# jizongFox/MI-based-Regularized-Semi-supervised-Segmentation

Measured on AMD Instinct MI355X. Metric: images/sec (UNet+IIC fwd/bwd) ACDC 256^2, higher is better.
Workload: dtype bf16; 1 GPU; udaiic train step, ACDC-shaped 1x256x256 4-class slices, LB=UB=16 per GPU, taps Conv5/Up_conv3/Up_conv2, K=20 x 5 sub-heads, paddings [1,3] (BASELINE configs[1]); mi_precision=f16f8, global_batch=32, parallelism=dp1, launch_tape=True, tape_ops=170, tape_replays_in_run=449

## Files before the change

include/miseg_hip.h:

```cpp
#ifndef MISEG_HIP_H
#define MISEG_HIP_H

#include <stdint.h>

#ifdef __cplusplus
extern "C" {
#endif

#define MISEG_F32 0
#define MISEG_BF16 1
#define MISEG_F16 2

#define MISEG_OK 0
#define MISEG_E_INVALID (-1)
#define MISEG_E_LAUNCH (-2)

int miseg_version(void);
const char* miseg_last_error(void);
int miseg_stream_wait_stream(void* waiter, void* producer);

int64_t miseg_tape_begin(void);
int miseg_tape_end(int64_t tape);
int miseg_tape_free(int64_t tape);
int64_t miseg_tape_mark(int64_t tape);
// ... 34 lines not shown
                        const float* grad_raw, const float* scale, float* gx, float* gy, int accumulate, int precision,
                        void* ws, int64_t ws_bytes);
int64_t miseg_iic_local_bwd_ws_bytes(int64_t K, int64_t pad, int64_t P);
int64_t miseg_iic_out_joint_ws_bytes(int64_t N, int64_t C, int64_t H, int64_t W, int64_t pad, int64_t P);
int miseg_iic_out_joint_fwd(void* stream, const float* a, const float* b, const int32_t* flips, int64_t N, int64_t C, int64_t H,
                            int64_t W, int64_t pad, const int32_t* win, int64_t P, float* raw, void* ws, int64_t ws_bytes);
int miseg_iic_out_bwd(void* stream, const float* a, const float* b, const int32_t* flips, int64_t N, int64_t C, int64_t H, int64_t W,
                      int64_t pad, const int32_t* win, int64_t P, const float* grad_raw, const float* scale, float* ga, float* gb,
                      int accumulate);
int miseg_iic_local_joint_fwd_heads(void* stream, const float* probs, int64_t S, int64_t UB, int64_t K, int64_t H, int64_t W,
                                    int64_t pad, const int32_t* win, int64_t P, float* raw, void* ws, int64_t ws_bytes,
                                    int precision);
int miseg_iic_local_bwd_heads(void* stream, const float* probs, int64_t S, int64_t UB, int64_t K, int64_t H, int64_t W,
                              int64_t pad, const int32_t* win, int64_t P, const float* grad_raw, const float* scale,
                              float* gprob, int accumulate, int precision, void* ws, int64_t ws_bytes);
int64_t miseg_iic_local_planes_bytes(int64_t S, int64_t UB, int64_t K, int64_t H, int64_t W, int64_t pad);
int miseg_iic_local_make_planes(void* stream, const float* probs, int64_t S, int64_t UB, int64_t K, int64_t H, int64_t W, int64_t pad,
                                void* planes, int64_t planes_bytes);
int miseg_iic_local_joint_fwd_heads_planes(void* stream, const float* probs, int64_t S, int64_t UB, int64_t K, int64_t H, int64_t W,
                                           int64_t pad, const int32_t* win, int64_t P, float* raw, void* ws, int64_t ws_bytes,
                                           void* planes, int64_t planes_bytes);
int miseg_iic_local_bwd_heads_planes(void* stream, const void* planes, int64_t planes_bytes, int64_t S, int64_t UB, int64_t K, int64_t H,
                                     int64_t W, int64_t pad, const int32_t* win, int64_t P, const float* grad_raw, const float* scale,
                                     float* gprob, int accumulate, void* ws, int64_t ws_bytes);

int miseg_iic_global_fwd(void* stream, const float* x, const float* y, int64_t S, int64_t N, int64_t K,
                         float lamb, float* loss, float* loss_no_lamb, float* joint);
int miseg_iic_global_bwd(void* stream, const float* x, const float* y, int64_t S, int64_t N, int64_t K,
                         float lamb, const float* upstream, float* gx, float* gy);
int miseg_iic_global_fwd_pair(void* stream, const float* prob, int64_t S, int64_t N, int64_t K, float lamb, float* loss,
// ... 223 lines not shown
```

mi-based-regularized-semi-supervised-segmentation_amd/csrc/api.hip:

```cpp
#include <stdarg.h>

#include "common.h"

namespace miseg_core {
static thread_local char g_err[512] = "";
char* last_error_buf() { return g_err; }
int fail(int code, const char* fmt, ...) {
    va_list ap;
    va_start(ap, fmt);
    vsnprintf(g_err, sizeof(g_err), fmt, ap);
    va_end(ap);
    return code;
}
}

extern "C" int miseg_version(void) { return 406; }
extern "C" const char* miseg_last_error(void) { return miseg::last_error_buf(); }

namespace miseg_core {
static hipEvent_t next_fork_event() {
    constexpr int kRing = 256, kDev = 16;
    struct Ring { hipEvent_t ev[kRing]; int made = 0, next = 0; };
    static thread_local Ring rings[kDev];
    int dev = 0;
    if (hipGetDevice(&dev) != hipSuccess || dev < 0 || dev >= kDev) return nullptr;
    Ring& r = rings[dev];
    constexpr unsigned flags = hipEventDisableTiming | hipEventDisableSystemFence;
    if (r.made < kRing) {
        if (hipEventCreateWithFlags(&r.ev[r.made], flags) != hipSuccess) return nullptr;
        ++r.made;
    }
// ... 17 lines not shown
```

mi-based-regularized-semi-supervised-segmentation_amd/csrc/mi_local.h:

```cpp
#pragma once
#include "common.h"

namespace miseg {

constexpr int kThreads = 256;
constexpr int kLdsBudget = 156 * 1024;

struct JointGeom {
    int N, K, H, W, pad, T, Mdim;
    int RB, WB, RW;
    int WX, RBY;
    int planeX, planeY;
    int P, G;
    int tilesM, sb, tps;
    int S;
    long long hs;
};

constexpr int kJT = 512;

template <int MT, int NT, int ROLE>
struct TileSet {
    static constexpr int SPLIT = (MT * NT + 1) / 2;
    static constexpr bool mine(int m, int n) { return ((m * NT + n) < SPLIT) == (ROLE == 0); }
// ... 53 lines not shown
#ifdef __HIPCC__
__device__ __forceinline__ unsigned pack_fp8x4(float a, float b, float c, float d) {
    int w = __builtin_amdgcn_cvt_pk_fp8_f32(a, b, 0, false);
    w = __builtin_amdgcn_cvt_pk_fp8_f32(c, d, w, true);
    return (unsigned)w;
}

__device__ __forceinline__ void split_quad(const float* v, qu32x2& h16, unsigned& l8, unsigned& h8) {
    const qh2_t h01 = {(_Float16)v[0], (_Float16)v[1]}, h23 = {(_Float16)v[2], (_Float16)v[3]};
    h16 = qu32x2{__builtin_bit_cast(unsigned, h01), __builtin_bit_cast(unsigned, h23)};
    l8 = pack_fp8x4((v[0] - (float)h01[0]) * 1048576.f, (v[1] - (float)h01[1]) * 1048576.f, (v[2] - (float)h23[0]) * 1048576.f,
                    (v[3] - (float)h23[1]) * 1048576.f);
    h8 = pack_fp8x4(v[0] * 256.f, v[1] * 256.f, v[2] * 256.f, v[3] * 256.f);
}

#endif

struct MiPlanes {
    unsigned char *p16, *p8l, *p8h;
};
constexpr int64_t kPlaneSlack = 4096;
static inline int64_t mi_planes_bytes(int64_t maps, int64_t HW) { return maps * HW * 88 + 4 * kPlaneSlack; }
static inline MiPlanes mi_planes(unsigned char* base, int64_t maps, int64_t HW) {
    if (!base) return MiPlanes{nullptr, nullptr, nullptr};
    unsigned char* p16 = base + kPlaneSlack;
    unsigned char* p8l = p16 + maps * HW * 40 + kPlaneSlack;
    return MiPlanes{p16, p8l, p8l + maps * HW * 24 + kPlaneSlack};
}
int launch_make_planes(hipStream_t st, const float* probs, int64_t maps, int64_t HW, unsigned char* planes);
size_t local_bwd_f8_ws_bytes(int64_t K, int64_t pad, int64_t P);
int launch_local_bwd_f8(hipStream_t st, const float* x, const float* y, int64_t S, int64_t hs, int64_t N, int64_t K, int64_t H, int64_t W,
                        int64_t pad, const int32_t* win, int64_t P, const float* grad_raw, const float* scale, float* gx, float* gy,
                        int accumulate, void* ws, const unsigned char* planes);

int launch_local_bwd_rows(hipStream_t st, const float* x, const float* y, int64_t S, int64_t hs, int64_t N, int64_t K, int64_t H, int64_t W,
                          int64_t pad, const int32_t* win, int64_t P, const float* grad_raw, const float* scale, float* gx, float* gy,
                          int accumulate, void* ws, int nterms, const unsigned char* planes = nullptr);

}
```

mi-based-regularized-semi-supervised-segmentation_amd/csrc/mi_local.hip:

```cpp
#include "mi_local.h"

namespace miseg {

template <int MT, int NT, int ROLE>
__device__ __forceinline__ void joint_fwd_body(const float* __restrict__ x, const float* __restrict__ y,
                                               const float* __restrict__ mask, const JointGeom& g,
                                               const int32_t* __restrict__ win, float* __restrict__ partials, float* lds) {
    typedef TileSet<MT, NT, ROLE> TS;
    float* Xs = lds;
    float* Ys = lds + (size_t)g.K * g.planeX;
    const int tid = threadIdx.x, lane = tid & 63, pair = tid >> 7;
    const int l15 = lane & 15, kq = lane >> 4;
    const int slot = blockIdx.y;
    const int sn = slot % g.sb, sm = (slot / g.sb) % g.sb, p = slot / (g.sb * g.sb);
    const int mtu = min(g.tps, g.tilesM - sm * g.tps), ntu = min(g.tps, g.tilesM - sn * g.tps);
    const int h0 = win[p * 4 + 0], h1 = win[p * 4 + 1], w0 = win[p * 4 + 2], w1 = win[p * 4 + 3];
    const int tr = (h1 - h0 + g.RB - 1) / g.RB, tc = (w1 - w0 + g.WB - 1) / g.WB;
    const int nItems = g.N * tr * tc;

    int aoff[MT], boff[NT];
#pragma unroll
    for (int mt = 0; mt < MT; ++mt) {
        int m = min((sm * g.tps + mt) * 16 + l15, g.Mdim - 1);
        aoff[mt] = (m % g.K) * g.planeX + (m / g.K) + kq;
// ... 95 lines not shown
                                                             const int32_t* __restrict__ win, float* __restrict__ partials) {
    extern __shared__ __attribute__((aligned(16))) float lds[];
    if (__builtin_amdgcn_readfirstlane(threadIdx.x >> 6) & 1) joint_fwd_body<MT, NT, 1>(x, y, mask, g, win, partials, lds);
    else joint_fwd_body<MT, NT, 0>(x, y, mask, g, win, partials, lds);
}

__global__ __launch_bounds__(256) void joint_reduce_kernel(const float* __restrict__ partials, JointGeom g, int MTmax, float* __restrict__ raw) {
    const int TT = g.T * g.T, KK = g.K * g.K;
    const int Dn = MTmax * 16, Dsz = Dn * Dn;
    reduce_partials_block(partials, g.G, (size_t)Dsz, g.P * TT * KK, raw, [=](int e) {
        const int j = e % g.K, i = (e / g.K) % g.K, b = (e / KK) % g.T, a = (e / (KK * g.T)) % g.T, p = e / (KK * TT);
        const int m = b * g.K + i, c = a * g.K + j;
        const int sm = m / (g.tps * 16), sn = c / (g.tps * 16);
        return ((size_t)((p * g.sb + sm) * g.sb + sn) * g.G) * Dsz + (size_t)(m - sm * g.tps * 16) * Dn + (c - sn * g.tps * 16);
    });
}

__device__ __forceinline__ float loss_displacement(const float* __restrict__ Rg, float mn, int K, int TT, float lamda, float* Pw,
                                                   float* Gw, float* colv, float* rowv, float* __restrict__ grad_d, int lane) {
    const int KK = K * K;
    const float eps = 1e-16f;
    float* Rw = rowv + 3 * K;
    for (int e = lane; e < KK; e += 64) Rw[e] = Rg[e];
    __builtin_amdgcn_wave_barrier();
    __threadfence_block();
    const float* R = Rw;
    float z = 0.f;
    for (int e = lane; e < KK; e += 64) z += (R[e] - mn) + eps;
    z = wave_sum(z);
    for (int e = lane; e < KK; e += 64) {
        int i = e / K, j = e % K;
        float q = ((R[e] - mn) + eps) / z, qt = ((R[j * K + i] - mn) + eps) / z;
        Pw[e] = (q + qt) / 2.0f;
    }
    __builtin_amdgcn_wave_barrier();
    __threadfence_block();
    if (K <= 32) {
        const int c = lane & 31;
        if (c < K) {
            float v = 0.f;
            if (lane < 32) { for (int t = 0; t < K; ++t) v += Pw[t * K + c]; }
            else { for (int t = 0; t < K; ++t) v += Pw[c * K + t]; }
            float* o = lane < 32 ? colv : rowv;
            o[c] = logf(v + eps);
            o[2 * K + c] = v / (v + eps);
        }
    } else {
        for (int c = lane; c < K; c += 64) {
            float cs = 0.f, rs = 0.f;
            for (int t = 0; t < K; ++t) { cs += Pw[t * K + c]; rs += Pw[c * K + t]; }
            colv[c] = logf(cs + eps), colv[2 * K + c] = cs / (cs + eps);
            rowv[c] = logf(rs + eps), rowv[2 * K + c] = rs / (rs + eps);
        }
    }
    __builtin_amdgcn_wave_barrier();
    __threadfence_block();
    float part = 0.f;
    for (int e = lane; e < KK; e += 64) {
        int i = e / K, j = e % K;
        float ps = Pw[e];
        float lp = logf(ps + eps), lc = colv[j], lr = rowv[i];
        part += ps * (lp - lamda * lc - lamda * lr);
        Gw[e] = -(lp + ps / (ps + eps) - lamda * (lc + colv[2 * K + j]) - lamda * (lr + rowv[2 * K + i])) / (float)TT;
    }
    const float term = -wave_sum(part);
    __builtin_amdgcn_wave_barrier();
    __threadfence_block();
    float sdot = 0.f;
    for (int e = lane; e < KK; e += 64) {
        int i = e / K, j = e % K;
        float gq = (Gw[e] + Gw[j * K + i]) / 2.0f;
        float q = ((R[e] - mn) + eps) / z;
        sdot += gq * q;
    }
    sdot = wave_sum(sdot);
    for (int e = lane; e < KK; e += 64) {
        int i = e / K, j = e % K;
        float gq = (Gw[e] + Gw[j * K + i]) / 2.0f;
        grad_d[e] = (gq - sdot) / z;
    }
    __builtin_amdgcn_wave_barrier();
    __threadfence_block();
    return term;
}

__global__ __launch_bounds__(1024) void local_loss_kernel(const float* __restrict__ raw_all, int K, int T, float lamda,
                                                          float* __restrict__ loss, float* __restrict__ grad_all) {
    extern __shared__ __attribute__((aligned(16))) float sm[];
    __shared__ float red[17];
    const int KK = K * K, TT = T * T, nw = blockDim.x >> 6, wid = threadIdx.x >> 6, lane = threadIdx.x & 63;
    const float* raw = raw_all + (size_t)blockIdx.x * TT * KK;
    float* grad = grad_all + (size_t)blockIdx.x * TT * KK;
    float* Pw = sm + (size_t)wid * (3 * KK + 4 * K);
    float* Gw = Pw + KK;
    float* colv = Gw + KK;
    float* rowv = colv + K;
    float mn = 3.4e38f;
    for (int e = threadIdx.x; e < TT * KK; e += blockDim.x) mn = fminf(mn, raw[e]);
// ... 520 lines not shown
                                           float* loss, float* grad_raw, void* ws, int64_t ws_bytes) {
    MISEG_TAPE(miseg_iic_local_loss_fwd_ws, stream, raw, K, pad, P, lamda, loss, grad_raw, ws, ws_bytes);
    MISEG_REQUIRE(raw && loss && grad_raw && ws, "iic_local_loss_fwd_ws: null pointer");
    MISEG_REQUIRE(K > 0 && K <= 64 && pad >= 0 && P > 0, "iic_local_loss_fwd_ws: bad shape");
    MISEG_REQUIRE(ws_bytes >= miseg_iic_local_loss_ws_bytes(pad, P), "iic_local_loss_fwd_ws: workspace too small");
    const int T = 2 * (int)pad + 1;
    const size_t ldsb = (size_t)(3 * K * K + 4 * K) * 4;
    hipLaunchKernelGGL(local_loss_disp_kernel, dim3((unsigned)P, (unsigned)(T * T)), dim3(1024), ldsb, as_stream(stream), raw, (int)K, T,
                       lamda, (float*)ws, grad_raw);
    MISEG_LAUNCH_CHECK("local_loss_disp_kernel");
    hipLaunchKernelGGL(local_loss_finish_kernel, dim3((unsigned)P), dim3(64), 0, as_stream(stream), (const float*)ws, T * T, loss);
    MISEG_LAUNCH_CHECK("local_loss_finish_kernel");
    return MISEG_OK;
}

extern "C" int miseg_iic_local_loss_fwd(void* stream, const float* raw, int64_t K, int64_t pad, int64_t P, float lamda,
                                        float* loss, float* grad_raw) {
    MISEG_TAPE(miseg_iic_local_loss_fwd, stream, raw, K, pad, P, lamda, loss, grad_raw);
    MISEG_REQUIRE(raw && loss && grad_raw, "iic_local_loss_fwd: null pointer");
    MISEG_REQUIRE(K > 0 && K <= 64 && pad >= 0 && P > 0, "iic_local_loss_fwd: bad shape");
    const int T = 2 * (int)pad + 1;
    const size_t ldsb = (size_t)16 * (3 * K * K + 4 * K) * 4;
    MISEG_REQUIRE(ldsb <= (size_t)kLdsBudget, "iic_local_loss_fwd: K too large");
    hipFuncSetAttribute((const void*)local_loss_kernel, hipFuncAttributeMaxDynamicSharedMemorySize, (int)ldsb);
    hipLaunchKernelGGL(local_loss_kernel, dim3((unsigned)P), dim3(1024), ldsb, as_stream(stream), raw, (int)K, T, lamda, loss,
                       grad_raw);
    MISEG_LAUNCH_CHECK("local_loss_kernel");
    return MISEG_OK;
}

// ... 69 lines not shown
```

mi-based-regularized-semi-supervised-segmentation_amd/csrc/mi_local_bwd_f8.hip:

```cpp
#include "mi_local.h"

#ifndef MISEG_F8_D1
#define MISEG_F8_D1 1
#endif
#ifndef MISEG_F8_BQ
#define MISEG_F8_BQ 1
#endif
#ifndef MISEG_F8_EDGE1
#define MISEG_F8_EDGE1 1
#endif
#ifndef MISEG_F8_STAMP
#define MISEG_F8_STAMP 0
#endif
#ifndef MISEG_F8_STORE_AUX
#define MISEG_F8_STORE_AUX 0
#endif
#ifndef MISEG_F8_ABL
#define MISEG_F8_ABL 0
#endif

namespace miseg {

template <int K, int PAD, int NT_ = 4>
struct Q3 {
// ... 1 lines not shown
    static constexpr int T = 2 * PAD + 1, REM = K - 16, RT = (T * REM + 15) / 16, MT = T + RT, MP = MT * 16;
    static constexpr int KRED = T * K, KS = (KRED + 31) / 32;
    static constexpr int CS8 = 24, CH = (T * CS8 + 31) / 32, NI = (2 * CH + 3) / 4;
    static constexpr int NT = NT_, WT = 16 * NT_, WS = WT + 2 * PAD, WSP = (WS + 7) / 8 * 8, CS = K;
    static constexpr int B16P = WSP * CS * 2;
    static constexpr int B8P = (((WT - 1) * CS8 + CH * 32 > WS * CS8 ? (WT - 1) * CS8 + CH * 32 : WS * CS8) + 15) / 16 * 16;
    static constexpr int A16B = KS * MP * 64, A8B = NI * 8 * MP * 16;
    static_assert(MP % 16 == 0, "A8 bank pattern");
};

struct Rows8Geom {
    int N, H, W, P, S, accumulate, G;
    long long hs;
};

__global__ __launch_bounds__(1024) void gexp_kernel(const float* __restrict__ grad_raw, int per, float* __restrict__ gexp) {
    const float* G = grad_raw + (size_t)blockIdx.x * per;
    float m = 0.f;
    for (int e = threadIdx.x; e < per; e += 1024) m = fmaxf(m, fabsf(G[e]));
#pragma unroll
    for (int o = 32; o > 0; o >>= 1) m = fmaxf(m, __shfl_xor(m, o, 64));
    __shared__ float red[16];
    if ((threadIdx.x & 63) == 0) red[threadIdx.x >> 6] = m;
    __syncthreads();
    if (threadIdx.x == 0) {
#pragma unroll
        for (int i = 1; i < 16; ++i) m = fmaxf(m, red[i]);
        gexp[blockIdx.x] = (m > 0.f && m < 3.0e38f) ? ldexpf(1.f, ilogbf(m)) : 1.f;
    }
}

__global__ __launch_bounds__(256) void make_planes_kernel(const float* __restrict__ probs, int maps, int HW, unsigned char* __restrict__ p16,
                                                          unsigned char* __restrict__ p8l, unsigned char* __restrict__ p8h) {
    constexpr int K = 20;
    const int pix = blockIdx.x * 256 + threadIdx.x, map = blockIdx.y;
    if (pix >= HW || map >= maps) return;
    const float* src = probs + (size_t)map * K * HW + pix;
    const size_t at = (size_t)map * HW + pix;
    unsigned h[10], l[6], g[6];
#pragma unroll
    for (int c4 = 0; c4 < K; c4 += 4) {
        const float v[4] = {src[(size_t)c4 * HW], src[(size_t)(c4 + 1) * HW], src[(size_t)(c4 + 2) * HW], src[(size_t)(c4 + 3) * HW]};
        qu32x2 hh;
// ... 6 lines not shown
    for (int i = 0; i < 5; ++i) o16[i] = qu32x2{h[2 * i], h[2 * i + 1]};
    qu32x2* ol = reinterpret_cast<qu32x2*>(p8l + at * 24);
    qu32x2* oh = reinterpret_cast<qu32x2*>(p8h + at * 24);
#pragma unroll
    for (int i = 0; i < 3; ++i) ol[i] = qu32x2{l[2 * i], l[2 * i + 1]}, oh[i] = qu32x2{g[2 * i], g[2 * i + 1]};
}

__device__ __forceinline__ void glds16(const void* gsrc, unsigned lds_dst) {
    unsigned keep;
    asm volatile("s_mov_b32 %0, m0\n\ts_mov_b32 m0, %2\n\ts_nop 0\n\tglobal_load_lds_dwordx4 %1, off\n\ts_mov_b32 m0, %0"
                 : "=&s"(keep) : "v"(gsrc), "s"(lds_dst) : "memory");
}
template <int N> __device__ __forceinline__ void wait_vm() { asm volatile("s_waitcnt vmcnt(%0)" ::"n"(N) : "memory"); }

template <int K, int PAD>
__device__ __forceinline__ float g_value(const float* __restrict__ grad_raw, int p, int dir, int m, int beta, int c, float inv) {
    typedef Q3<K, PAD> C;
    int tau, o;
    if (m < C::T * 16) { tau = m >> 4; o = m & 15; }
    else { const int rr = m - C::T * 16; tau = rr / C::REM; o = 16 + rr % C::REM; }
    if (tau >= C::T || beta >= C::T || c >= K) return 0.f;
    const int a = dir ? tau : C::T - 1 - tau, b = dir ? beta : C::T - 1 - beta;
    const float* G = grad_raw + (size_t)p * C::T * C::T * K * K + (size_t)(a * C::T + b) * K * K;
    return (dir ? G[c * K + o] : G[o * K + c]) * inv;
}

template <int K, int PAD>
__global__ void pack_g_f8_kernel(const float* __restrict__ grad_raw, const float* __restrict__ gexp, int PS, unsigned char* __restrict__ gpack) {
    typedef Q3<K, PAD> C;
    constexpr int N16 = C::KS * C::MP * 32, N8 = C::NI * 8 * C::MP * 4;
    const int total = PS * 2 * (N16 + N8);
    for (int e = blockIdx.x * blockDim.x + threadIdx.x; e < total; e += gridDim.x * blockDim.x) {
        const int sdp = e / (N16 + N8), r = e - sdp * (N16 + N8), dir = sdp & 1, p = sdp >> 1;
        const float inv = 1.f / gexp[p];
        unsigned char* base = gpack + (size_t)sdp * (C::A16B + C::A8B);
        if (r < N16) {
            const int kk = r & 31, m = (r >> 5) % C::MP, ks = r / (32 * C::MP);
            const int kred = ks * 32 + kk;
            const float v = kred < C::KRED ? g_value<K, PAD>(grad_raw, p, dir, m, kred / K, kred % K, inv) : 0.f;
            const _Float16 h = (_Float16)v;
            const size_t at = ((size_t)ks * C::MP + m) * 32 + 8 * ((kk >> 3) ^ ((0 - (m >> 2)) & 3)) + (kk & 7);
            reinterpret_cast<_Float16*>(base)[at] = h;
        } else {
            const int d = r - N16, b4 = d & 3, chunk = (d >> 6) & 7, m = ((d >> 9) % C::MT) * 16 + ((d >> 2) & 15), t = d / (512 * C::MT);
            const int j = 4 * t + (chunk >> 1), term = j / C::CH;
            float v[4];
#pragma unroll
            for (int i = 0; i < 4; ++i) {
                const int byte = (chunk & 1) * 16 + b4 * 4 + i, kk = (j % C::CH) * 32 + byte;
                float g = j < 2 * C::CH ? g_value<K, PAD>(grad_raw, p, dir, m, kk / C::CS8, kk % C::CS8, inv) : 0.f;
                const float h = (float)(_Float16)g;
                v[i] = term == 0 ? h * 128.f : (g - h) * 524288.f;
            }
            reinterpret_cast<unsigned*>(base + C::A16B)[d] = pack_fp8x4(v[0], v[1], v[2], v[3]);
        }
    }
}

template <int K, int PAD, bool ACC, int NTW, int WAVES, bool PL>
__global__ __launch_bounds__(64 * WAVES, 1) void local_bwd_f8_kernel(const float* __restrict__ x, const float* __restrict__ y, Rows8Geom g,
                                                              const int32_t* __restrict__ win,
                                                              const unsigned char* __restrict__ gpack, const float* __restrict__ gexp,
                                                              const float* __restrict__ scale, float* __restrict__ gx,
                                                              float* __restrict__ gy, unsigned long long* __restrict__ stamps,
                                                              const unsigned char* __restrict__ pl16, const unsigned char* __restrict__ pl8l,
                                                              const unsigned char* __restrict__ pl8h) {
    typedef Q3<K, PAD, NTW> C;
    constexpr int T = C::T, RT = C::RT, NT = C::NT, KS = C::KS, NI = C::NI, MP = C::MP, CS = C::CS, CS8 = C::CS8;
    constexpr int BWB = C::B16P + 2 * C::B8P;
    extern __shared__ __attribute__((aligned(16))) unsigned char ldsb[];
// ... 376 lines not shown
    if (lane == 0) {
        unsigned long long* o = stamps + ((size_t)blockIdx.x * WAVES + wv) * 8;
        o[0] = st_fetch; o[1] = st_p1; o[2] = st_p2; o[3] = st_out; o[4] = st_rows;
    }
#endif
}

size_t local_bwd_f8_ws_bytes(int64_t K, int64_t pad, int64_t P) {
    if (K != 20 || pad != 3) return 0;
    typedef Q3<20, 3> C;
    return (size_t)256 + (size_t)((P * 4 + 255) / 256 * 256) + (size_t)P * 2 * (C::A16B + C::A8B) + (MISEG_F8_STAMP ? 256 * 8 * 64 : 0);
}

bool local_bwd_f8_supported(int64_t K, int64_t pad) { return K == 20 && pad == 3; }

int launch_local_bwd_f8(hipStream_t st, const float* x, const float* y, int64_t S, int64_t hs, int64_t N, int64_t K, int64_t H, int64_t W,
                        int64_t pad, const int32_t* win, int64_t P, const float* grad_raw, const float* scale, float* gx, float* gy,
                        int accumulate, void* ws, const unsigned char* planes) {
    typedef Q3<20, 3, 4> C;
    constexpr int WAVES = 8;
    Rows8Geom g{(int)N, (int)H, (int)W, (int)P, (int)S, accumulate, 256, (long long)hs};
    const int PS = (int)(P * S);
    float* gexp = reinterpret_cast<float*>(ws);
    unsigned char* gpack = reinterpret_cast<unsigned char*>(ws) + (size_t)((PS * 4 + 255) / 256 * 256);
    hipLaunchKernelGGL(gexp_kernel, dim3(PS), dim3(1024), 0, st, grad_raw, C::T * C::T * 20 * 20, gexp);
    const int total = PS * 2 * (C::KS * C::MP * 32 + C::NI * 8 * C::MP * 4);
    hipLaunchKernelGGL((pack_g_f8_kernel<20, 3>), dim3((total + 255) / 256), dim3(256), 0, st, grad_raw, gexp, PS, gpack);
    const size_t lds = (size_t)C::A16B + C::A8B + (size_t)WAVES * (C::B16P + 2 * C::B8P);
    const MiPlanes pl = mi_planes(const_cast<unsigned char*>(planes), S * 2 * N, H * W);
    auto go = [&](auto kernel) {
        hipFuncSetAttribute((const void*)kernel, hipFuncAttributeMaxDynamicSharedMemorySize, (int)lds);
        hipLaunchKernelGGL(kernel, dim3(g.G), dim3(64 * WAVES), lds, st, x, y, g, win, gpack, gexp, scale, gx, gy,
                           reinterpret_cast<unsigned long long*>(gpack + (size_t)PS * 2 * (C::A16B + C::A8B)), pl.p16, pl.p8l, pl.p8h);
    };
    if (planes) {
        if (g.accumulate) go(local_bwd_f8_kernel<20, 3, true, 4, WAVES, true>);
        else go(local_bwd_f8_kernel<20, 3, false, 4, WAVES, true>);
    } else {
        if (g.accumulate) go(local_bwd_f8_kernel<20, 3, true, 4, WAVES, false>);
        else go(local_bwd_f8_kernel<20, 3, false, 4, WAVES, false>);
    }
    return 0;
}

int launch_make_planes(hipStream_t st, const float* probs, int64_t maps, int64_t HW, unsigned char* planes) {
    const MiPlanes pl = mi_planes(planes, maps, HW);
    hipLaunchKernelGGL(make_planes_kernel, dim3((unsigned)((HW + 255) / 256), (unsigned)maps), dim3(256), 0, st, probs, (int)maps, (int)HW, pl.p16, pl.p8l,
                       pl.p8h);
    return 0;
}

}
```

mi-based-regularized-semi-supervised-segmentation_amd/miseg_amd/ops.py:

```python
from __future__ import annotations

import os
from typing import List, Optional, Sequence, Tuple

import torch
from torch import Tensor

from . import _cabi, stepio
from ._cabi import BF16, F16, F32, call, query
from .tape import keep

_DT = {torch.float32: F32, torch.bfloat16: BF16, torch.float16: F16}


_raw_stream = getattr(torch._C, "_cuda_getCurrentRawStream", None)
_raw_device = getattr(torch._C, "_cuda_getDevice", None)


def _stream() -> int:
    if _raw_stream is not None and _raw_device is not None:
        return _raw_stream(_raw_device())
    return torch.cuda.current_stream().cuda_stream


# ... 200 lines not shown
        whole = _is_whole(ctx.windows, h, w)
        gx, gy = (torch.empty_like(x), torch.empty_like(y)) if whole else (torch.zeros_like(x), torch.zeros_like(y))
        _local_bwd(x, y, mask, ctx.pad, ctx.windows, win, grad_raw, gloss.contiguous().float(), gx, gy)
        return gx, gy, None, None, None, None


def _local_loss(raw: Tensor, k: int, pad: int, p: int, lamda: float, loss: Tensor, grad_raw: Tensor) -> None:
    if pad >= 2:
        ws = _ws(query("miseg_iic_local_loss_ws_bytes", pad, p), raw.device)
        call("miseg_iic_local_loss_fwd_ws", _stream(), _ptr(raw), k, pad, p, float(lamda), _ptr(loss), _ptr(grad_raw), _ptr(ws), ws.numel())
    else:
        call("miseg_iic_local_loss_fwd", _stream(), _ptr(raw), k, pad, p, float(lamda), _ptr(loss), _ptr(grad_raw))


_MI_PLANES = os.environ.get("MISEG_MI_PLANES", "0") == "1"


class _LocalMIHeads(torch.autograd.Function):

    @staticmethod
    def forward(ctx, probs: Tensor, ub: int, mask: Optional[Tensor], pad: int, windows, lamda: float):
        _need_gpu(probs, mask)
        probs = probs.contiguous().float()
        mask = None if mask is None else mask.contiguous().float()
        s, n2, k, h, w = probs.shape
        if n2 != 2 * ub:
            raise _cabi.MisegError(f"local_mi_heads: probs holds {n2} maps per sub-head, expected 2*{ub}")
        p, t, dev = len(windows), 2 * pad + 1, probs.device
        win = windows_tensor(windows, dev)
        raw = torch.empty(s, p, t, t, k, k, dtype=torch.float32, device=dev)
# ... 4 lines not shown
            px = sum((a1 - a0) * (b1 - b0) for a0, a1, b0, b1 in windows)
            nplanes = query("miseg_iic_local_planes_bytes", s, ub, k, h, w, pad) if _MI_PLANES and _mi_precision == MI_PRECISIONS["f16f8"] else 0
            if nplanes > 0:
                planes = torch.empty(nplanes, dtype=torch.uint8, device=dev)
                call("miseg_iic_local_joint_fwd_heads_planes", _stream(), _ptr(probs), s, ub, k, h, w, pad, _ptr(win), p, _ptr(raw), _ptr(ws),
                     ws.numel(), _ptr(planes), nplanes, work=(2.0 * k * k * t * t * ub * px * s, 2.0 * ub * k * px * (4 + 4.4) * s),
                     tag=f"iic_local_joint_fwd[p{pad}]")
            else:
                call("miseg_iic_local_joint_fwd_heads", _stream(), _ptr(probs), s, ub, k, h, w, pad, _ptr(win), p, _ptr(raw), _ptr(ws), ws.numel(),
                     _mi_precision, work=(2.0 * k * k * t * t * ub * px * s, 2.0 * ub * k * px * 4 * s), tag=f"iic_local_joint_fwd[p{pad}]")
        else:
            for i in range(s):
                _local_fwd(probs[i, :ub], probs[i, ub:], mask, pad, windows, win, raw[i])
        loss = scalar_out((s, p), dev)
        grad_raw = torch.empty_like(raw)
        _local_loss(raw, k, pad, s * p, lamda, loss, grad_raw)
        ctx.save_for_backward(planes if planes is not None else probs, mask, grad_raw, win)
        ctx.pad, ctx.windows, ctx.ub, ctx.planes, ctx.shape = pad, list(windows), ub, planes is not None, tuple(probs.shape)
        return loss

    @staticmethod
    def backward(ctx, gloss: Tensor):
        probs, mask, grad_raw, win = ctx.saved_tensors
        s, _, k, h, w = ctx.shape
        ub = ctx.ub
        gprob = torch.empty(ctx.shape, dtype=torch.float32, device=probs.device)
        if not _is_whole(ctx.windows, h, w):
            fill_zero(gprob)
        scale = gloss.contiguous().float()
        if mask is None:
            whole = _is_whole(ctx.windows, h, w)
            tt = (2 * ctx.pad + 1) ** 2
            bws = _ws(query("miseg_iic_local_bwd_ws_bytes", k, ctx.pad, len(ctx.windows) * s), probs.device)
            for grp in colour_windows(ctx.windows):
                if len(grp) == len(ctx.windows):
                    gwin, ggrad, gscale = win, grad_raw, scale
                else:
                    dev = probs.device
                    idx = cached_const(("idx32", str(dev), tuple(grp)), lambda: torch.tensor(grp, dtype=torch.int32, device=dev))
                    gwin = cached_const(("gwin", str(dev), tuple(ctx.windows), tuple(grp)), lambda: win[idx.long()].contiguous())
                    npw, per = len(ctx.windows), grad_raw[0, 0].numel()
                    ggrad = torch.empty((s, len(grp)) + tuple(grad_raw.shape[2:]), dtype=torch.float32, device=dev)
                    gscale = torch.empty((s, len(grp)), dtype=torch.float32, device=dev)
                    call("miseg_gather_rows", _stream(), _ptr(grad_raw), _ptr(ggrad), s, npw, len(grp), _ptr(idx), per)
                    call("miseg_gather_rows", _stream(), _ptr(scale), _ptr(gscale), s, npw, len(grp), _ptr(idx), 1)
# ... 731 lines not shown
```

Baseline: 4949 images/s.

## Fuse local MI loss with f8 gradient packing and skip backward pre-pack kernels

Adds a loss_pack kernel that computes the local IIC loss and its gradient and, in the same launch, writes the per-(head,window) gradient exponent and the f16/f8-packed gradient tiles into a saved buffer. Backward then calls a packed entry point that goes straight to the f8 bwd kernel, dropping the separate gexp and pack_g kernel launches and a reread of grad_raw. It applies only for K=20, pad=3, f16f8 precision with planes off and a single colour group, and it keeps an extra pack buffer alive from forward to backward.

```diff
diff --git a/include/miseg_hip.h b/include/miseg_hip.h
--- a/include/miseg_hip.h
+++ b/include/miseg_hip.h
@@ -72,6 +72,12 @@
 int miseg_iic_local_bwd_heads(void* stream, const float* probs, int64_t S, int64_t UB, int64_t K, int64_t H, int64_t W,
                               int64_t pad, const int32_t* win, int64_t P, const float* grad_raw, const float* scale,
                               float* gprob, int accumulate, int precision, void* ws, int64_t ws_bytes);
+int64_t miseg_iic_local_loss_pack_bytes(int64_t S, int64_t UB, int64_t K, int64_t H, int64_t W, int64_t pad, int64_t P);
+int miseg_iic_local_loss_pack(void* stream, const float* raw, int64_t K, int64_t pad, int64_t PS, float lamda, float* loss,
+                              float* grad_raw, void* ws, int64_t ws_bytes, void* pack, int64_t pack_bytes);
+int miseg_iic_local_bwd_heads_packed(void* stream, const float* probs, int64_t S, int64_t UB, int64_t K, int64_t H, int64_t W,
+                                     int64_t pad, const int32_t* win, int64_t P, const void* pack, int64_t pack_bytes,
+                                     const float* scale, float* gprob, int accumulate);
 int64_t miseg_iic_local_planes_bytes(int64_t S, int64_t UB, int64_t K, int64_t H, int64_t W, int64_t pad);
 int miseg_iic_local_make_planes(void* stream, const float* probs, int64_t S, int64_t UB, int64_t K, int64_t H, int64_t W, int64_t pad,
                                 void* planes, int64_t planes_bytes);
diff --git a/mi-based-regularized-semi-supervised-segmentation_amd/csrc/api.hip b/mi-based-regularized-semi-supervised-segmentation_amd/csrc/api.hip
--- a/mi-based-regularized-semi-supervised-segmentation_amd/csrc/api.hip
+++ b/mi-based-regularized-semi-supervised-segmentation_amd/csrc/api.hip
@@ -14,7 +14,7 @@
 }
 }
 
-extern "C" int miseg_version(void) { return 406; }
+extern "C" int miseg_version(void) { return 407; }
 extern "C" const char* miseg_last_error(void) { return miseg::last_error_buf(); }
 
 namespace miseg_core {
diff --git a/mi-based-regularized-semi-supervised-segmentation_amd/csrc/mi_local.h b/mi-based-regularized-semi-supervised-segmentation_amd/csrc/mi_local.h
--- a/mi-based-regularized-semi-supervised-segmentation_amd/csrc/mi_local.h
+++ b/mi-based-regularized-semi-supervised-segmentation_amd/csrc/mi_local.h
@@ -91,6 +91,74 @@
     h8 = pack_fp8x4(v[0] * 256.f, v[1] * 256.f, v[2] * 256.f, v[3] * 256.f);
 }
 
+__device__ __forceinline__ float loss_displacement(const float* __restrict__ Rg, float mn, int K, int TT, float lamda, float* Pw,
+                                                   float* Gw, float* colv, float* rowv, float* __restrict__ grad_d, int lane) {
+    const int KK = K * K;
+    const float eps = 1e-16f;
+    float* Rw = rowv + 3 * K;
+    for (int e = lane; e < KK; e += 64) Rw[e] = Rg[e];
+    __builtin_amdgcn_wave_barrier();
+    __threadfence_block();
+    const float* R = Rw;
+    float z = 0.f;
+    for (int e = lane; e < KK; e += 64) z += (R[e] - mn) + eps;
+    z = wave_sum(z);
+    for (int e = lane; e < KK; e += 64) {
+        int i = e / K, j = e % K;
+        float q = ((R[e] - mn) + eps) / z, qt = ((R[j * K + i] - mn) + eps) / z;
+        Pw[e] = (q + qt) / 2.0f;
+    }
+    __builtin_amdgcn_wave_barrier();
+    __threadfence_block();
+    if (K <= 32) {
+        const int c = lane & 31;
+        if (c < K) {
+            float v = 0.f;
+            if (lane < 32) { for (int t = 0; t < K; ++t) v += Pw[t * K + c]; }
+            else { for (int t = 0; t < K; ++t) v += Pw[c * K + t]; }
+            float* o = lane < 32 ? colv : rowv;
+            o[c] = logf(v + eps);
+            o[2 * K + c] = v / (v + eps);
+        }
+    } else {
+        for (int c = lane; c < K; c += 64) {
+            float cs = 0.f, rs = 0.f;
+            for (int t = 0; t < K; ++t) { cs += Pw[t * K + c]; rs += Pw[c * K + t]; }
+            colv[c] = logf(cs + eps), colv[2 * K + c] = cs / (cs + eps);
+            rowv[c] = logf(rs + eps), rowv[2 * K + c] = rs / (rs + eps);
+        }
+    }
+    __builtin_amdgcn_wave_barrier();
+    __threadfence_block();
+    float part = 0.f;
+    for (int e = lane; e < KK; e += 64) {
+        int i = e / K, j = e % K;
+        float ps = Pw[e];
+        float lp = logf(ps + eps), lc = colv[j], lr = rowv[i];
+        part += ps * (lp - lamda * lc - lamda * lr);
+        Gw[e] = -(lp + ps / (ps + eps) - lamda * (lc + colv[2 * K + j]) - lamda * (lr + rowv[2 * K + i])) / (float)TT;
+    }
+    const float term = -wave_sum(part);
+    __builtin_amdgcn_wave_barrier();
+    __threadfence_block();
+    float sdot = 0.f;
+    for (int e = lane; e < KK; e += 64) {
+        int i = e / K, j = e % K;
+        float gq = (Gw[e] + Gw[j * K + i]) / 2.0f;
+        float q = ((R[e] - mn) + eps) / z;
+        sdot += gq * q;
+    }
+    sdot = wave_sum(sdot);
+    for (int e = lane; e < KK; e += 64) {
+        int i = e / K, j = e % K;
+        float gq = (Gw[e] + Gw[j * K + i]) / 2.0f;
+        grad_d[e] = (gq - sdot) / z;
+    }
+    __builtin_amdgcn_wave_barrier();
+    __threadfence_block();
+    return term;
+}
+
 #endif
 
 struct MiPlanes {
@@ -110,6 +178,10 @@
                         int64_t pad, const int32_t* win, int64_t P, const float* grad_raw, const float* scale, float* gx, float* gy,
                         int accumulate, void* ws, const unsigned char* planes);
 
+int launch_local_bwd_f8_packed(hipStream_t st, const float* x, const float* y, int64_t S, int64_t hs, int64_t N, int64_t H, int64_t W, const int32_t* win,
+                               int64_t P, const void* ws, const float* scale, float* gx, float* gy, int accumulate, const unsigned char* planes);
+int launch_loss_pack_f8(hipStream_t st, const float* raw, int64_t PS, float lamda, float* loss, float* parts, float* grad_raw, void* pack);
+
 int launch_local_bwd_rows(hipStream_t st, const float* x, const float* y, int64_t S, int64_t hs, int64_t N, int64_t K, int64_t H, int64_t W,
                           int64_t pad, const int32_t* win, int64_t P, const float* grad_raw, const float* scale, float* gx, float* gy,
                           int accumulate, void* ws, int nterms, const unsigned char* planes = nullptr);
diff --git a/mi-based-regularized-semi-supervised-segmentation_amd/csrc/mi_local.hip b/mi-based-regularized-semi-supervised-segmentation_amd/csrc/mi_local.hip
--- a/mi-based-regularized-semi-supervised-segmentation_amd/csrc/mi_local.hip
+++ b/mi-based-regularized-semi-supervised-segmentation_amd/csrc/mi_local.hip
@@ -133,74 +133,6 @@
         const int sm = m / (g.tps * 16), sn = c / (g.tps * 16);
         return ((size_t)((p * g.sb + sm) * g.sb + sn) * g.G) * Dsz + (size_t)(m - sm * g.tps * 16) * Dn + (c - sn * g.tps * 16);
     });
-}
-
-__device__ __forceinline__ float loss_displacement(const float* __restrict__ Rg, float mn, int K, int TT, float lamda, float* Pw,
-                                                   float* Gw, float* colv, float* rowv, float* __restrict__ grad_d, int lane) {
-    const int KK = K * K;
-    const float eps = 1e-16f;
-    float* Rw = rowv + 3 * K;
-    for (int e = lane; e < KK; e += 64) Rw[e] = Rg[e];
-    __builtin_amdgcn_wave_barrier();
-    __threadfence_block();
-    const float* R = Rw;
-    float z = 0.f;
-    for (int e = lane; e < KK; e += 64) z += (R[e] - mn) + eps;
-    z = wave_sum(z);
-    for (int e = lane; e < KK; e += 64) {
-        int i = e / K, j = e % K;
-        float q = ((R[e] - mn) + eps) / z, qt = ((R[j * K + i] - mn) + eps) / z;
-        Pw[e] = (q + qt) / 2.0f;
-    }
-    __builtin_amdgcn_wave_barrier();
-    __threadfence_block();
-    if (K <= 32) {
-        const int c = lane & 31;
-        if (c < K) {
-            float v = 0.f;
-            if (lane < 32) { for (int t = 0; t < K; ++t) v += Pw[t * K + c]; }
-            else { for (int t = 0; t < K; ++t) v += Pw[c * K + t]; }
-            float* o = lane < 32 ? colv : rowv;
-            o[c] = logf(v + eps);
-            o[2 * K + c] = v / (v + eps);
-        }
-    } else {
-        for (int c = lane; c < K; c += 64) {
-            float cs = 0.f, rs = 0.f;
-            for (int t = 0; t < K; ++t) { cs += Pw[t * K + c]; rs += Pw[c * K + t]; }
-            colv[c] = logf(cs + eps), colv[2 * K + c] = cs / (cs + eps);
-            rowv[c] = logf(rs + eps), rowv[2 * K + c] = rs / (rs + eps);
-        }
-    }
-    __builtin_amdgcn_wave_barrier();
-    __threadfence_block();
-    float part = 0.f;
-    for (int e = lane; e < KK; e += 64) {
-        int i = e / K, j = e % K;
-        float ps = Pw[e];
-        float lp = logf(ps + eps), lc = colv[j], lr = rowv[i];
-        part += ps * (lp - lamda * lc - lamda * lr);
-        Gw[e] = -(lp + ps / (ps + eps) - lamda * (lc + colv[2 * K + j]) - lamda * (lr + rowv[2 * K + i])) / (float)TT;
-    }
-    const float term = -wave_sum(part);
-    __builtin_amdgcn_wave_barrier();
-    __threadfence_block();
-    float sdot = 0.f;
-    for (int e = lane; e < KK; e += 64) {
-        int i = e / K, j = e % K;
-        float gq = (Gw[e] + Gw[j * K + i]) / 2.0f;
-        float q = ((R[e] - mn) + eps) / z;
-        sdot += gq * q;
-    }
-    sdot = wave_sum(sdot);
-    for (int e = lane; e < KK; e += 64) {
-        int i = e / K, j = e % K;
-        float gq = (Gw[e] + Gw[j * K + i]) / 2.0f;
-        grad_d[e] = (gq - sdot) / z;
-    }
-    __builtin_amdgcn_wave_barrier();
-    __threadfence_block();
-    return term;
 }
 
 __global__ __launch_bounds__(1024) void local_loss_kernel(const float* __restrict__ raw_all, int K, int T, float lamda,
@@ -751,6 +683,41 @@
     return MISEG_OK;
 }
 
+extern "C" int64_t miseg_iic_local_loss_pack_bytes(int64_t S, int64_t UB, int64_t K, int64_t H, int64_t W, int64_t pad, int64_t P) {
+    if (S <= 0 || UB <= 0 || H <= 0 || W <= 0 || P <= 0 || !local_bwd_f8_supported(K, pad) || !local_bwd_bf16_supported(UB, K, H, W, pad)) return 0;
+    if (P * S > 32) return 0;
+    return (int64_t)local_bwd_f8_ws_bytes(K, pad, P * S);
+}
+
+extern "C" int miseg_iic_local_loss_pack(void* stream, const float* raw, int64_t K, int64_t pad, int64_t PS, float lamda, float* loss,
+                                         float* grad_raw, void* ws, int64_t ws_bytes, void* pack, int64_t pack_bytes) {
+    MISEG_TAPE(miseg_iic_local_loss_pack, stream, raw, K, pad, PS, lamda, loss, grad_raw, ws, ws_bytes, pack, pack_bytes);
+    MISEG_REQUIRE(raw && loss && grad_raw && ws && pack, "iic_local_loss_pack: null pointer");
+    MISEG_REQUIRE(local_bwd_f8_supported(K, pad) && PS > 0 && PS <= 32, "iic_local_loss_pack: K = 20, pad = 3, at most 32 (sub-head, window) pairs");
+    MISEG_REQUIRE(ws_bytes >= miseg_iic_local_loss_ws_bytes(pad, PS), "iic_local_loss_pack: workspace too small");
+    MISEG_REQUIRE(pack_bytes >= (int64_t)local_bwd_f8_ws_bytes(K, pad, PS), "iic_local_loss_pack: pack buffer %ld < %ld", (long)pack_bytes,
+                  (long)local_bwd_f8_ws_bytes(K, pad, PS));
+    MISEG_REQUIRE((reinterpret_cast<uintptr_t>(raw) & 15) == 0 && (reinterpret_cast<uintptr_t>(grad_raw) & 15) == 0 &&
+                  (reinterpret_cast<uintptr_t>(pack) & 15) == 0, "iic_local_loss_pack: raw, grad_raw and pack must be 16-byte aligned");
+    launch_loss_pack_f8(as_stream(stream), raw, PS, lamda, loss, (float*)ws, grad_raw, pack);
+    MISEG_LAUNCH_CHECK("loss_pack_f8_kernel");
+    return MISEG_OK;
+}
+
+extern "C" int miseg_iic_local_bwd_heads_packed(void* stream, const float* probs, int64_t S, int64_t UB, int64_t K, int64_t H, int64_t W,
+                                                int64_t pad, const int32_t* win, int64_t P, const void* pack, int64_t pack_bytes,
+                                                const float* scale, float* gprob, int accumulate) {
+    MISEG_TAPE(miseg_iic_local_bwd_heads_packed, stream, probs, S, UB, K, H, W, pad, win, P, pack, pack_bytes, scale, gprob, accumulate);
+    MISEG_REQUIRE(probs && win && pack && scale && gprob, "iic_local_bwd_heads_packed: null pointer");
+    const int64_t need = miseg_iic_local_loss_pack_bytes(S, UB, K, H, W, pad, P);
+    MISEG_REQUIRE(need > 0, "iic_local_bwd_heads_packed: shape not supported (K = 20, pad = 3)");
+    MISEG_REQUIRE(pack_bytes >= need, "iic_local_bwd_heads_packed: pack buffer %ld < %ld", (long)pack_bytes, (long)need);
+    const int64_t hs = 2 * UB * K * H * W, half = UB * K * H * W;
+    launch_local_bwd_f8_packed(as_stream(stream), probs, probs + half, S, hs, UB, H, W, win, P, pack, scale, gprob, gprob + half, accumulate, nullptr);
+    MISEG_LAUNCH_CHECK("local_bwd_f8_kernel");
+    return MISEG_OK;
+}
+
 extern "C" int miseg_iic_local_loss_fwd(void* stream, const float* raw, int64_t K, int64_t pad, int64_t P, float lamda,
                                         float* loss, float* grad_raw) {
     MISEG_TAPE(miseg_iic_local_loss_fwd, stream, raw, K, pad, P, lamda, loss, grad_raw);
diff --git a/mi-based-regularized-semi-supervised-segmentation_amd/csrc/mi_local_bwd_f8.hip b/mi-based-regularized-semi-supervised-segmentation_amd/csrc/mi_local_bwd_f8.hip
--- a/mi-based-regularized-semi-supervised-segmentation_amd/csrc/mi_local_bwd_f8.hip
+++ b/mi-based-regularized-semi-supervised-segmentation_amd/csrc/mi_local_bwd_f8.hip
@@ -39,6 +39,8 @@
     long long hs;
 };
 
+__device__ __forceinline__ float gexp_of(float m) { return (m > 0.f && m < 3.0e38f) ? ldexpf(1.f, ilogbf(m)) : 1.f; }
+
 __global__ __launch_bounds__(1024) void gexp_kernel(const float* __restrict__ grad_raw, int per, float* __restrict__ gexp) {
     const float* G = grad_raw + (size_t)blockIdx.x * per;
     float m = 0.f;
@@ -51,7 +53,7 @@
     if (threadIdx.x == 0) {
 #pragma unroll
         for (int i = 1; i < 16; ++i) m = fmaxf(m, red[i]);
-        gexp[blockIdx.x] = (m > 0.f && m < 3.0e38f) ? ldexpf(1.f, ilogbf(m)) : 1.f;
+        gexp[blockIdx.x] = gexp_of(m);
     }
 }
 
@@ -88,15 +90,41 @@
 template <int N> __device__ __forceinline__ void wait_vm() { asm volatile("s_waitcnt vmcnt(%0)" ::"n"(N) : "memory"); }
 
 template <int K, int PAD>
-__device__ __forceinline__ float g_value(const float* __restrict__ grad_raw, int p, int dir, int m, int beta, int c, float inv) {
+__device__ __forceinline__ float g_value(const float* __restrict__ G, int dir, int m, int beta, int c, float inv) {
     typedef Q3<K, PAD> C;
     int tau, o;
     if (m < C::T * 16) { tau = m >> 4; o = m & 15; }
     else { const int rr = m - C::T * 16; tau = rr / C::REM; o = 16 + rr % C::REM; }
     if (tau >= C::T || beta >= C::T || c >= K) return 0.f;
     const int a = dir ? tau : C::T - 1 - tau, b = dir ? beta : C::T - 1 - beta;
-    const float* G = grad_raw + (size_t)p * C::T * C::T * K * K + (size_t)(a * C::T + b) * K * K;
-    return (dir ? G[c * K + o] : G[o * K + c]) * inv;
+    const float* Gd = G + (size_t)(a * C::T + b) * K * K;
+    return (dir ? Gd[c * K + o] : Gd[o * K + c]) * inv;
+}
+
+template <int K, int PAD>
+__device__ __forceinline__ void pack_g_item(const float* __restrict__ G, float inv, int dir, int r, unsigned char* __restrict__ base) {
+    typedef Q3<K, PAD> C;
+    constexpr int N16 = C::KS * C::MP * 32;
+    if (r < N16) {
+        const int kk = r & 31, m = (r >> 5) % C::MP, ks = r / (32 * C::MP);
+        const int kred = ks * 32 + kk;
+        const float v = kred < C::KRED ? g_value<K, PAD>(G, dir, m, kred / K, kred % K, inv) : 0.f;
+        const _Float16 h = (_Float16)v;
+        const size_t at = ((size_t)ks * C::MP + m) * 32 + 8 * ((kk >> 3) ^ ((0 - (m >> 2)) & 3)) + (kk & 7);
+        reinterpret_cast<_Float16*>(base)[at] = h;
+    } else {
+        const int d = r - N16, b4 = d & 3, chunk = (d >> 6) & 7, m = ((d >> 9) % C::MT) * 16 + ((d >> 2) & 15), t = d / (512 * C::MT);
+        const int j = 4 * t + (chunk >> 1), term = j / C::CH;
+        float v[4];
+#pragma unroll
+        for (int i = 0; i < 4; ++i) {
+            const int byte = (chunk & 1) * 16 + b4 * 4 + i, kk = (j % C::CH) * 32 + byte;
+            float g = j < 2 * C::CH ? g_value<K, PAD>(G, dir, m, kk / C::CS8, kk % C::CS8, inv) : 0.f;
+            const float h = (float)(_Float16)g;
+            v[i] = term == 0 ? h * 128.f : (g - h) * 524288.f;
+        }
+        reinterpret_cast<unsigned*>(base + C::A16B)[d] = pack_fp8x4(v[0], v[1], v[2], v[3]);
+    }
 }
 
 template <int K, int PAD>
@@ -107,27 +135,71 @@
     for (int e = blockIdx.x * blockDim.x + threadIdx.x; e < total; e += gridDim.x * blockDim.x) {
         const int sdp = e / (N16 + N8), r = e - sdp * (N16 + N8), dir = sdp & 1, p = sdp >> 1;
         const float inv = 1.f / gexp[p];
-        unsigned char* base = gpack + (size_t)sdp * (C::A16B + C::A8B);
-        if (r < N16) {
-            const int kk = r & 31, m = (r >> 5) % C::MP, ks = r / (32 * C::MP);
-            const int kred = ks * 32 + kk;
-            const float v = kred < C::KRED ? g_value<K, PAD>(grad_raw, p, dir, m, kred / K, kred % K, inv) : 0.f;
-            const _Float16 h = (_Float16)v;
-            const size_t at = ((size_t)ks * C::MP + m) * 32 + 8 * ((kk >> 3) ^ ((0 - (m >> 2)) & 3)) + (kk & 7);
-            reinterpret_cast<_Float16*>(base)[at] = h;
-        } else {
-            const int d = r - N16, b4 = d & 3, chunk = (d >> 6) & 7, m = ((d >> 9) % C::MT) * 16 + ((d >> 2) & 15), t = d / (512 * C::MT);
-            const int j = 4 * t + (chunk >> 1), term = j / C::CH;
-            float v[4];
-#pragma unroll
-            for (int i = 0; i < 4; ++i) {
-                const int byte = (chunk & 1) * 16 + b4 * 4 + i, kk = (j % C::CH) * 32 + byte;
-                float g = j < 2 * C::CH ? g_value<K, PAD>(grad_raw, p, dir, m, kk / C::CS8, kk % C::CS8, inv) : 0.f;
-                const float h = (float)(_Float16)g;
-                v[i] = term == 0 ? h * 128.f : (g - h) * 524288.f;
-            }
-            reinterpret_cast<unsigned*>(base + C::A16B)[d] = pack_fp8x4(v[0], v[1], v[2], v[3]);
+        pack_g_item<K, PAD>(grad_raw + (size_t)p * C::T * C::T * K * K, inv, dir, r, gpack + (size_t)sdp * (C::A16B + C::A8B));
+    }
+}
+
+constexpr int kLossPackNB = 8, kLossPackWaves = 16;
+template <int K, int PAD>
+__global__ __launch_bounds__(64 * kLossPackWaves) void loss_pack_f8_kernel(const float* __restrict__ raw_all, float lamda, float* __restrict__ loss,
+                                                                           float* __restrict__ parts, float* __restrict__ grad_all,
+                                                                           float* __restrict__ gexp, unsigned char* __restrict__ gpack) {
+    typedef Q3<K, PAD> C;
+    constexpr int KK = K * K, TT = C::T * C::T, PER = TT * KK, WSCR = 3 * KK + 4 * K;
+    constexpr int N16 = C::KS * C::MP * 32, N8 = C::NI * 8 * C::MP * 4, NTH = 64 * kLossPackWaves;
+    static_assert(PER % 4 == 0, "16-byte pieces of the joint");
+    extern __shared__ __attribute__((aligned(16))) float lp_sm[];
+    __shared__ float red[17];
+    __shared__ float terms[(TT + 63) / 64 * 64];
+    float* Gs = lp_sm;
+    const int tid = threadIdx.x, wid = tid >> 6, lane = tid & 63, sp = blockIdx.x;
+    const bool writer = blockIdx.y == 0;
+    const float* raw = raw_all + (size_t)sp * PER;
+    float mn = 3.4e38f;
+    for (int e = tid; e < PER / 4; e += NTH) {
+        const float4 v = reinterpret_cast<const float4*>(raw)[e];
+        mn = fminf(fminf(mn, v.x), fminf(fminf(v.y, v.z), v.w));
+    }
+    mn = block_min(mn, red);
+    {
+        float* Pw = lp_sm + PER + (size_t)wid * WSCR;
+        float* Gw = Pw + KK;
+        float* colv = Gw + KK;
+        float* rowv = colv + K;
+        for (int d = wid; d < TT; d += kLossPackWaves) {
+            const float term = loss_displacement(raw + (size_t)d * KK, mn, K, TT, lamda, Pw, Gw, colv, rowv, Gs + (size_t)d * KK, lane);
+            if (lane == 0) terms[d] = term;
         }
+    }
+    __syncthreads();
+    float m = 0.f;
+    for (int e = tid; e < PER; e += NTH) m = fmaxf(m, fabsf(Gs[e]));
+#pragma unroll
+    for (int o = 32; o > 0; o >>= 1) m = fmaxf(m, __shfl_xor(m, o, 64));
+    if (lane == 0) red[wid] = m;
+    __syncthreads();
+#pragma unroll
+    for (int i = 0; i < kLossPackWaves; ++i) m = fmaxf(m, red[i]);
+    const float ge = gexp_of(m);
+    if (writer) {
+        if (tid == 0) gexp[sp] = ge;
+        float* grad = grad_all + (size_t)sp * PER;
+        for (int e = tid; e < PER / 4; e += NTH) reinterpret_cast<float4*>(grad)[e] = reinterpret_cast<const float4*>(Gs)[e];
+        if (wid == 0) {
+            float tot = 0.f;
+            for (int d0 = 0; d0 < TT; d0 += 64) {
+                const float v = d0 + lane < TT ? terms[d0 + lane] : 0.f;
+                if (d0 + lane < TT) parts[(size_t)sp * TT + d0 + lane] = v;
+                const int mm = min(64, TT - d0);
+                for (int d = 0; d < mm; ++d) tot += __shfl(v, d, 64);
+            }
+            if (lane == 0) loss[sp] = tot / (float)TT;
+        }
+    }
+    const float inv = 1.f / ge;
+    for (int e = blockIdx.y * NTH + tid; e < 2 * (N16 + N8); e += kLossPackNB * NTH) {
+        const int dir = e >= N16 + N8, r = e - dir * (N16 + N8);
+        pack_g_item<K, PAD>(Gs, inv, dir, r, gpack + (size_t)(sp * 2 + dir) * (C::A16B + C::A8B));
     }
 }
 
@@ -534,23 +606,22 @@
 
 bool local_bwd_f8_supported(int64_t K, int64_t pad) { return K == 20 && pad == 3; }
 
-int launch_local_bwd_f8(hipStream_t st, const float* x, const float* y, int64_t S, int64_t hs, int64_t N, int64_t K, int64_t H, int64_t W,
-                        int64_t pad, const int32_t* win, int64_t P, const float* grad_raw, const float* scale, float* gx, float* gy,
-                        int accumulate, void* ws, const unsigned char* planes) {
+static inline float* f8_ws_gexp(void* ws) { return reinterpret_cast<float*>(ws); }
+static inline unsigned char* f8_ws_gpack(void* ws, int PS) { return reinterpret_cast<unsigned char*>(ws) + (size_t)((PS * 4 + 255) / 256 * 256); }
+
+int launch_local_bwd_f8_packed(hipStream_t st, const float* x, const float* y, int64_t S, int64_t hs, int64_t N, int64_t H, int64_t W, const int32_t* win,
+                               int64_t P, const void* ws, const float* scale, float* gx, float* gy, int accumulate, const unsigned char* planes) {
     typedef Q3<20, 3, 4> C;
     constexpr int WAVES = 8;
     Rows8Geom g{(int)N, (int)H, (int)W, (int)P, (int)S, accumulate, 256, (long long)hs};
     const int PS = (int)(P * S);
-    float* gexp = reinterpret_cast<float*>(ws);
-    unsigned char* gpack = reinterpret_cast<unsigned char*>(ws) + (size_t)((PS * 4 + 255) / 256 * 256);
-    hipLaunchKernelGGL(gexp_kernel, dim3(PS), dim3(1024), 0, st, grad_raw, C::T * C::T * 20 * 20, gexp);
-    const int total = PS * 2 * (C::KS * C::MP * 32 + C::NI * 8 * C::MP * 4);
-    hipLaunchKernelGGL((pack_g_f8_kernel<20, 3>), dim3((total + 255) / 256), dim3(256), 0, st, grad_raw, gexp, PS, gpack);
+    const float* gexp = f8_ws_gexp(const_cast<void*>(ws));
+    unsigned char* gpack = f8_ws_gpack(const_cast<void*>(ws), PS);
     const size_t lds = (size_t)C::A16B + C::A8B + (size_t)WAVES * (C::B16P + 2 * C::B8P);
     const MiPlanes pl = mi_planes(const_cast<unsigned char*>(planes), S * 2 * N, H * W);
     auto go = [&](auto kernel) {
         hipFuncSetAttribute((const void*)kernel, hipFuncAttributeMaxDynamicSharedMemorySize, (int)lds);
-        hipLaunchKernelGGL(kernel, dim3(g.G), dim3(64 * WAVES), lds, st, x, y, g, win, gpack, gexp, scale, gx, gy,
+        hipLaunchKernelGGL(kernel, dim3(g.G), dim3(64 * WAVES), lds, st, x, y, g, win, (const unsigned char*)gpack, gexp, scale, gx, gy,
                            reinterpret_cast<unsigned long long*>(gpack + (size_t)PS * 2 * (C::A16B + C::A8B)), pl.p16, pl.p8l, pl.p8h);
     };
     if (planes) {
@@ -563,6 +634,27 @@
     return 0;
 }
 
+int launch_local_bwd_f8(hipStream_t st, const float* x, const float* y, int64_t S, int64_t hs, int64_t N, int64_t K, int64_t H, int64_t W,
+                        int64_t pad, const int32_t* win, int64_t P, const float* grad_raw, const float* scale, float* gx, float* gy,
+                        int accumulate, void* ws, const unsigned char* planes) {
+    typedef Q3<20, 3, 4> C;
+    const int PS = (int)(P * S);
+    float* gexp = f8_ws_gexp(ws);
+    hipLaunchKernelGGL(gexp_kernel, dim3(PS), dim3(1024), 0, st, grad_raw, C::T * C::T * 20 * 20, gexp);
+    const int total = PS * 2 * (C::KS * C::MP * 32 + C::NI * 8 * C::MP * 4);
+    hipLaunchKernelGGL((pack_g_f8_kernel<20, 3>), dim3((total + 255) / 256), dim3(256), 0, st, grad_raw, (const float*)gexp, PS, f8_ws_gpack(ws, PS));
+    return launch_local_bwd_f8_packed(st, x, y, S, hs, N, H, W, win, P, ws, scale, gx, gy, accumulate, planes);
+}
+
+int launch_loss_pack_f8(hipStream_t st, const float* raw, int64_t PS, float lamda, float* loss, float* parts, float* grad_raw, void* pack) {
+    typedef Q3<20, 3> C;
+    const size_t lds = (size_t)(C::T * C::T * 400 + kLossPackWaves * (3 * 400 + 4 * 20)) * 4;
+    hipFuncSetAttribute((const void*)loss_pack_f8_kernel<20, 3>, hipFuncAttributeMaxDynamicSharedMemorySize, (int)lds);
+    hipLaunchKernelGGL((loss_pack_f8_kernel<20, 3>), dim3((unsigned)PS, kLossPackNB), dim3(64 * kLossPackWaves), lds, st, raw, lamda, loss, parts,
+                       grad_raw, f8_ws_gexp(pack), f8_ws_gpack(pack, (int)PS));
+    return 0;
+}
+
 int launch_make_planes(hipStream_t st, const float* probs, int64_t maps, int64_t HW, unsigned char* planes) {
     const MiPlanes pl = mi_planes(planes, maps, HW);
     hipLaunchKernelGGL(make_planes_kernel, dim3((unsigned)((HW + 255) / 256), (unsigned)maps), dim3(256), 0, st, probs, (int)maps, (int)HW, pl.p16, pl.p8l,
diff --git a/mi-based-regularized-semi-supervised-segmentation_amd/miseg_amd/ops.py b/mi-based-regularized-semi-supervised-segmentation_amd/miseg_amd/ops.py
--- a/mi-based-regularized-semi-supervised-segmentation_amd/miseg_amd/ops.py
+++ b/mi-based-regularized-semi-supervised-segmentation_amd/miseg_amd/ops.py
@@ -238,6 +238,9 @@
 
 
 _MI_PLANES = os.environ.get("MISEG_MI_PLANES", "0") == "1"
+
+
+_LOSS_PACK = os.environ.get("MISEG_LOSS_PACK", "1") != "0"
 
 
 class _LocalMIHeads(torch.autograd.Function):
@@ -272,21 +275,37 @@
                 _local_fwd(probs[i, :ub], probs[i, ub:], mask, pad, windows, win, raw[i])
         loss = scalar_out((s, p), dev)
         grad_raw = torch.empty_like(raw)
-        _local_loss(raw, k, pad, s * p, lamda, loss, grad_raw)
-        ctx.save_for_backward(planes if planes is not None else probs, mask, grad_raw, win)
+        npack = 0
+        if _LOSS_PACK and mask is None and planes is None and _mi_precision == MI_PRECISIONS["f16f8"] and len(colour_windows(windows)) == 1:
+            npack = query("miseg_iic_local_loss_pack_bytes", s, ub, k, h, w, pad, p)
+        pack = None
+        if npack > 0:
+            pack = torch.empty(npack, dtype=torch.uint8, device=dev)
+            lws = _ws(query("miseg_iic_local_loss_ws_bytes", pad, s * p), dev)
+            call("miseg_iic_local_loss_pack", _stream(), _ptr(raw), k, pad, s * p, float(lamda), _ptr(loss), _ptr(grad_raw), _ptr(lws), lws.numel(),
+                 _ptr(pack), npack)
+        else:
+            _local_loss(raw, k, pad, s * p, lamda, loss, grad_raw)
+        ctx.save_for_backward(planes if planes is not None else probs, mask, grad_raw, win, pack)
         ctx.pad, ctx.windows, ctx.ub, ctx.planes, ctx.shape = pad, list(windows), ub, planes is not None, tuple(probs.shape)
         return loss
 
     @staticmethod
     def backward(ctx, gloss: Tensor):
-        probs, mask, grad_raw, win = ctx.saved_tensors
+        probs, mask, grad_raw, win, pack = ctx.saved_tensors
         s, _, k, h, w = ctx.shape
         ub = ctx.ub
         gprob = torch.empty(ctx.shape, dtype=torch.float32, device=probs.device)
         if not _is_whole(ctx.windows, h, w):
             fill_zero(gprob)
         scale = gloss.contiguous().float()
-        if mask is None:
+        if pack is not None:
+            tt = (2 * ctx.pad + 1) ** 2
+            px = sum((a1 - a0) * (b1 - b0) for a0, a1, b0, b1 in ctx.windows)
+            call("miseg_iic_local_bwd_heads_packed", _stream(), _ptr(probs), s, ub, k, h, w, ctx.pad, _ptr(win), len(ctx.windows), _ptr(pack),
+                 pack.numel(), _ptr(scale), _ptr(gprob), 0 if _is_whole(ctx.windows, h, w) else 1,
+                 work=(4.0 * k * k * tt * ub * px * s, 4.0 * ub * k * px * 4 * s), tag=f"iic_local_bwd[p{ctx.pad}]")
+        elif mask is None:
             whole = _is_whole(ctx.windows, h, w)
             tt = (2 * ctx.pad + 1) ** 2
             bws = _ws(query("miseg_iic_local_bwd_ws_bytes", k, ctx.pad, len(ctx.windows) * s), probs.device)
```

Result: slower. 4868 images/s (-1.6%).
